# facebookresearch/videoseal

Hardware: AMD Instinct MI355X
Metric: frames/sec embed+extract 256-bit @768x768 (higher is better)
Workload: dtype f32 (2 x f16 operand split, 3 products on v_mfma_f32_32x32x16_f16, fp32 accumulate); 1 GPU; videoseal_1.0 256-bit, 32 frames 768x768 per GPU, image mode (embedder on every frame, full-res JND), embed + detect; card=videoseal_1.0, weights=random-init (seeded), no checkpoint offline, batch_per_gpu=32, mode=image

## Files before the change

### videoseal_amd/csrc/conv3x3_pl.hip

```cpp
#include <type_traits>

#include "conv_common.h"
#include "lds_dma.h"

int vs_splitk_epilogue(const vs_conv_desc_t& d, int M, hipStream_t st);

namespace {

using namespace vsconv;

constexpr int PT = 16, PPW = PT + 2, PPIX = PPW * PPW;
constexpr int PL_UNITS = PPIX * 2;
constexpr int P_DMAS = (2 * PL_UNITS + 63) / 64;
constexpr int P_BYTES = P_DMAS * 1024;
constexpr int Q_BYTES = 256 * 2 * 2 * 16;
constexpr int QX_OFF = 2 * P_BYTES;
constexpr int RING_OFF = QX_OFF + 2 * Q_BYTES;
constexpr int NRING = 6;

__device__ __forceinline__ void dma16(const char* gp, unsigned char* lds_base) { vs_lds_dma16(gp, lds_base); }
template <int N>
__device__ __forceinline__ void wait_vm() { asm volatile("s_waitcnt vmcnt(%0)" ::"n"(N) : "memory"); }

template <int TN>
__global__ __launch_bounds__(512, 2) void conv3x3_pl_kernel(const vs_conv_desc_t d, const int tiles_x, const int tiles_y, const int mtiles,
                                                            const int ntiles, const int cps) {
  using AR = Arith<2>;
  constexpr int TM = 2;
  constexpr int BN = 2 * TN * 32;
  constexpr int NG = BN / 32;
  constexpr int WBLK = 2048;
  constexpr int B_STAGE = NG * WBLK;
  __shared__ __attribute__((aligned(16))) unsigned char smem[RING_OFF + NRING * B_STAGE];
  unsigned char* const Bring = smem + RING_OFF;

  const int tid = threadIdx.x;
  const int lane = tid & 63;
  const int wave = __builtin_amdgcn_readfirstlane(tid >> 6);
  const int r = lane & 31, g = lane >> 5;

  const int bm = blockIdx.x % mtiles;
  const int bn = (blockIdx.x / mtiles) % ntiles;
  const int ks = blockIdx.x / (mtiles * ntiles);
  const int n0 = bn * BN;
  const int tx = bm % tiles_x;
  const int ty = (bm / tiles_x) % tiles_y;
  const int fb = bm / (tiles_x * tiles_y);
  const int y0 = ty * PT, x0 = tx * PT;

  const int spt_all = d.CinP / BK;
  const int sk = d.split_k > 1 ? d.split_k : 1;
  const bool p2_slice = sk > 1 && ks == sk;
  const int c_off = (sk > 1 && !p2_slice) ? ks * cps : 0;
  const int spt = p2_slice ? 0 : (sk > 1 ? min(cps, spt_all - c_off) : spt_all);
  const int n1 = 9 * spt;
  const int n2 = (d.in2_pl && (sk == 1 || p2_slice)) ? d.Cin2P / BK : 0;
  const int64_t Mpix = (int64_t)d.B * d.H * d.W;
  const int abl = VS_KERNEL_ABL(d);

  const int64_t cstride = Mpix * 32;
  const int pw = wave & 3;
  const int g0 = n0 / 32;
  const int ngroups = (d.N + 31) / 32;
  unsigned doff[6];
  unsigned pvalid = 0;
  int wdst[TN];
#pragma unroll
  for (int jj = 0; jj < TN; ++jj) {
    const int idx = pw * TN + jj;
    const int p = idx / NG, gi = idx - p * NG;
    wdst[jj] = __builtin_amdgcn_readfirstlane(p * (BN * 32) + gi * 1024);
  }
  auto weight_off = [&](const int nst) __attribute__((always_inline)) {
#pragma unroll
    for (int jj = 0; jj < TN; ++jj) {
      const int idx = pw * TN + jj;
      const int p = idx / NG, gi = idx - p * NG;
      const int gs = (g0 + gi) < ngroups ? g0 + gi : ngroups - 1;
      doff[jj] = (unsigned)(gs * nst) * WBLK + p * 1024 + lane * 16;
    }
  };
  const char* wbase = reinterpret_cast<const char*>(d.wt_blk) + (int64_t)c_off * 9 * WBLK;
  if (wave < 4) {
    weight_off(9 * spt_all);
  } else {
    const unsigned pstride = (unsigned)(spt_all * cstride);
#pragma unroll
    for (int j = 0; j < 6; ++j) {
      const int U = (pw + 4 * j) * 64 + lane;
      const int plane = U >= PL_UNITS ? 1 : 0;
      const int u = U - plane * PL_UNITS;
      const int q = u >> 1;
      const int py = q / PPW, px = q - py * PPW;
      const int hs = (u & 1) ^ (py & 1);
      const int iy = y0 - 1 + py, ix = x0 - 1 + px;
      const bool ok = U < 2 * PL_UNITS && iy >= 0 && iy < d.H && ix >= 0 && ix < d.W;
      doff[j] = ok ? plane * pstride + (unsigned)(((fb * d.H + iy) * d.W + ix) * 32 + hs * 16) : 0u;
      pvalid |= ok ? 1u << j : 0u;
      if (!ok && pw + 4 * j < P_DMAS) {
        *reinterpret_cast<u32x4*>(smem + (pw + 4 * j) * 1024 + lane * 16) = u32x4{0u, 0u, 0u, 0u};
        *reinterpret_cast<u32x4*>(smem + P_BYTES + (pw + 4 * j) * 1024 + lane * 16) = u32x4{0u, 0u, 0u, 0u};
      }
    }
  }
  int wstage = 0;
  auto dma_w2 = [&]() __attribute__((always_inline)) {
    unsigned char* st = Bring + wstage * B_STAGE;
#pragma unroll
    for (int jj = 0; jj < TN; ++jj) dma16(wbase + doff[jj], st + wdst[jj]);
    wbase += WBLK;
    wstage = wstage + 1 == NRING ? 0 : wstage + 1;
  };
  auto dma_w = [&](auto stagec) __attribute__((always_inline)) {
    unsigned char* st = Bring + decltype(stagec)::value * B_STAGE;
#pragma unroll
    for (int jj = 0; jj < TN; ++jj) dma16(wbase + doff[jj], st + wdst[jj]);
    wbase += WBLK;
  };
  const char* const inpl = reinterpret_cast<const char*>(d.in_pl);
  auto dma_patch2 = [&](const int cc, const int j0) __attribute__((always_inline)) {
    unsigned char* pb = smem + (cc & 1) * P_BYTES + pw * 1024;
    const char* cbase = inpl + (c_off + cc) * cstride;
#pragma unroll
    for (int jj = 0; jj < 2; ++jj) {
      const int j = j0 + jj;
      if (pw + 4 * j < P_DMAS) {
        if ((pvalid >> j) & 1) dma16(cbase + doff[j], pb + j * 4096);
      }
    }
  };
  auto qbuf = [&](const int c2) __attribute__((always_inline)) -> unsigned char* {
    const int b = c2 & 3;
    return smem + (b < 2 ? QX_OFF + b * Q_BYTES : (b - 2) * Q_BYTES);
  };
  const char* qbase = reinterpret_cast<const char*>(d.in2_pl);
  auto q_off = [&]() __attribute__((always_inline)) {
    const unsigned pstride2 = (unsigned)((d.Cin2P / BK) * cstride);
#pragma unroll
    for (int j = 0; j < 4; ++j) {
      const int U = (pw + 4 * j) * 64 + lane;
      const int plane = U >> 9;
      const int u = U & 511;
      const int p = u >> 1;
      const int hs = (u & 1) ^ ((p >> 3) & 1);
      const int iy = y0 + (p >> 4), ix = x0 + (p & 15);
      doff[j] = plane * pstride2 + (unsigned)(((fb * d.H + iy) * d.W + ix) * 32 + hs * 16);
    }
  };
  auto dma_q = [&](const int c2) __attribute__((always_inline)) {
    unsigned char* qb = qbuf(c2) + pw * 1024;
#pragma unroll
    for (int j = 0; j < 4; ++j) dma16(qbase + doff[j], qb + j * 4096);
    qbase += cstride;
  };

  const int wm = wave >> 1, wn = wave & 1;
  f32x16 acc[TM][TN];
#pragma unroll
  for (int i = 0; i < TM; ++i)
#pragma unroll
    for (int j = 0; j < TN; ++j)
#pragma unroll
      for (int e = 0; e < 16; ++e) acc[i][j][e] = 0.f;
  int q0[TM], p0[TM], prow[TM];
#pragma unroll
  for (int i = 0; i < TM; ++i) {
    p0[i] = (wm * TM + i) * 32 + r;
    q0[i] = (p0[i] >> 4) * PPW + (p0[i] & 15);
    prow[i] = (p0[i] >> 4) & 1;
  }
  const int b_frag = (wn * TN) * 1024 + (2 * r + (g ^ ((r >> 3) & 1))) * 16;

  struct Hi { bf16x8 a[TM]; bf16x8 b[TN]; };
  Hi H0, H1;
  bf16x8 lo_a[TM], lo_b[TN];
  auto b_ptr = [&](const int s) __attribute__((always_inline)) -> const unsigned char* { return Bring + (s % NRING) * B_STAGE + b_frag; };
  auto load_all2 = [&](Hi& H, const int c2) __attribute__((always_inline)) {
    const unsigned char* Bb = b_ptr(c2);
#pragma unroll
    for (int j = 0; j < TN; ++j) {
      H.b[j] = *reinterpret_cast<const bf16x8*>(Bb + j * 1024);
      lo_b[j] = *reinterpret_cast<const bf16x8*>(Bb + BN * 32 + j * 1024);
    }
    const unsigned char* Qs = qbuf(c2);
#pragma unroll
    for (int i = 0; i < TM; ++i) {
      const int ao = (2 * p0[i] + (g ^ ((p0[i] >> 3) & 1))) * 16;
      H.a[i] = *reinterpret_cast<const bf16x8*>(Qs + ao);
      lo_a[i] = *reinterpret_cast<const bf16x8*>(Qs + 512 * 16 + ao);
    }
  };
  auto mfma_q0 = [&](const Hi& H) __attribute__((always_inline)) {
#pragma unroll
    for (int i = 0; i < TM; ++i)
#pragma unroll
      for (int j = 0; j < TN; ++j) acc[i][j] = AR::mfma(H.b[j], lo_a[i], acc[i][j]);
  };
  auto mfma_q1 = [&](const Hi& H) __attribute__((always_inline)) {
#pragma unroll
    for (int i = 0; i < TM; ++i)
#pragma unroll
      for (int j = 0; j < TN; ++j) acc[i][j] = AR::mfma(lo_b[j], H.a[i], acc[i][j]);
  };
  auto mfma_q2 = [&](const Hi& H) __attribute__((always_inline)) {
#pragma unroll
    for (int i = 0; i < TM; ++i)
#pragma unroll
      for (int j = 0; j < TN; ++j) acc[i][j] = AR::mfma(H.b[j], H.a[i], acc[i][j]);
  };
  int ab[TM];
#pragma unroll
  for (int i = 0; i < TM; ++i) ab[i] = (2 * q0[i] + (g ^ prow[i])) * 16;
  auto ld_hi = [&](Hi& H, auto parc, auto tapc) __attribute__((always_inline)) {
    constexpr int PAR = decltype(parc)::value, TAP = decltype(tapc)::value;
    constexpr int ky = TAP / 3, kx = TAP % 3, STAGE = (PAR * 3 + TAP) % NRING;
    const unsigned char* Bb = Bring + STAGE * B_STAGE + b_frag;
#pragma unroll
    for (int j = 0; j < TN; ++j) H.b[j] = *reinterpret_cast<const bf16x8*>(Bb + j * 1024);
    const unsigned char* Ps = smem + PAR * P_BYTES + (ky * PPW + kx) * 32;
#pragma unroll
    for (int i = 0; i < TM; ++i) H.a[i] = *reinterpret_cast<const bf16x8*>(Ps + ((ky & 1) ? (ab[i] ^ 16) : ab[i]));
  };
  auto ld_alo = [&](auto parc, auto tapc) __attribute__((always_inline)) {
    constexpr int PAR = decltype(parc)::value, TAP = decltype(tapc)::value;
    constexpr int ky = TAP / 3, kx = TAP % 3;
    const unsigned char* Ps = smem + PAR * P_BYTES + PL_UNITS * 16 + (ky * PPW + kx) * 32;
#pragma unroll
    for (int i = 0; i < TM; ++i) lo_a[i] = *reinterpret_cast<const bf16x8*>(Ps + ((ky & 1) ? (ab[i] ^ 16) : ab[i]));
  };
  auto ld_blo = [&](auto parc, auto tapc) __attribute__((always_inline)) {
    constexpr int PAR = decltype(parc)::value, TAP = decltype(tapc)::value;
    constexpr int STAGE = (PAR * 3 + TAP) % NRING;
    const unsigned char* Bb = Bring + STAGE * B_STAGE + BN * 32 + b_frag;
#pragma unroll
    for (int j = 0; j < TN; ++j) lo_b[j] = *reinterpret_cast<const bf16x8*>(Bb + j * 1024);
  };
  using P0 = std::integral_constant<int, 0>;
  using P1 = std::integral_constant<int, 1>;
  auto tapstep = [&](auto parc, auto tapc, const int cc, const bool last) __attribute__((always_inline)) {
    constexpr int PAR = decltype(parc)::value, TAP = decltype(tapc)::value;
    constexpr bool ODD = ((PAR + TAP) & 1) != 0;
    const Hi& Hc = ODD ? H1 : H0;
    Hi& Hn = ODD ? H0 : H1;
    const int s = cc * 9 + TAP;
    mfma_q0(Hc);
    __builtin_amdgcn_sched_barrier(0);
    if (wave < 4) {
      if (s + NRING - 1 < n1) dma_w(std::integral_constant<int, (PAR * 3 + TAP + NRING - 1) % NRING>{});
    } else if constexpr (TAP < 3) {
      if (!last) dma_patch2(cc + 1, 2 * TAP);
    }
    if constexpr (TAP < 8) {
      ld_hi(Hn, parc, std::integral_constant<int, TAP + 1>{});
      ld_alo(parc, std::integral_constant<int, TAP + 1>{});
    } else if (!last) {
      ld_hi(Hn, std::integral_constant<int, 1 - PAR>{}, P0{});
      ld_alo(std::integral_constant<int, 1 - PAR>{}, P0{});
    }
    mfma_q1(Hc);
    __builtin_amdgcn_sched_barrier(0);
    if constexpr (TAP < 8) ld_blo(parc, std::integral_constant<int, TAP + 1>{});
    else if (!last) ld_blo(std::integral_constant<int, 1 - PAR>{}, P0{});
    mfma_q2(Hc);
    if (wave < 4) {
      if (s + NRING - 1 < n1) wait_vm<(NRING - 3) * TN>();
      else wait_vm<0>();
    } else if constexpr (TAP == 7) {
      if (!last) wait_vm<0>();
    }
    __builtin_amdgcn_s_waitcnt(0xC07F);
    __builtin_amdgcn_s_barrier();
  };
  auto chunk = [&](auto parc, const int cc) __attribute__((always_inline)) {
    const bool last = cc + 1 >= spt;
    tapstep(parc, std::integral_constant<int, 0>{}, cc, last);
    tapstep(parc, std::integral_constant<int, 1>{}, cc, last);
    tapstep(parc, std::integral_constant<int, 2>{}, cc, last);
    tapstep(parc, std::integral_constant<int, 3>{}, cc, last);
    tapstep(parc, std::integral_constant<int, 4>{}, cc, last);
    tapstep(parc, std::integral_constant<int, 5>{}, cc, last);
    tapstep(parc, std::integral_constant<int, 6>{}, cc, last);
    tapstep(parc, std::integral_constant<int, 7>{}, cc, last);
    tapstep(parc, std::integral_constant<int, 8>{}, cc, last);
  };

  if (spt > 0) {
  if (wave < 4) {
    dma_w(std::integral_constant<int, 0>{});
    dma_w(std::integral_constant<int, 1>{});
    dma_w(std::integral_constant<int, 2>{});
    dma_w(std::integral_constant<int, 3>{});
    dma_w(std::integral_constant<int, 4>{});
  } else {
    dma_patch2(0, 0);
    dma_patch2(0, 2);
    dma_patch2(0, 4);
  }
  wait_vm<0>();
  __builtin_amdgcn_s_barrier();

  ld_hi(H0, P0{}, P0{});
  ld_alo(P0{}, P0{});
  ld_blo(P0{}, P0{});
  __builtin_amdgcn_s_waitcnt(0xC07F);
  for (int cc = 0; cc < spt; cc += 2) {
    chunk(P0{}, cc);
    if (cc + 1 < spt) chunk(P1{}, cc + 1);
  }
  }
  int lane_e = lane;
  asm volatile("" : "+v"(lane_e));
  const int r_e = lane_e & 31, g_e = lane_e >> 5;
  int cbase[TN];
#pragma unroll
  for (int j = 0; j < TN; ++j) cbase[j] = n0 + (wn * TN + j) * 32 + 4 * g_e;
  auto ld4 = [](const float* p, int n, int N) __attribute__((always_inline)) -> f32x4 {
    f32x4 v = {0.f, 0.f, 0.f, 0.f};
    if (p) {
      if (n + 4 <= N) v = *reinterpret_cast<const f32x4*>(p + n);
      else
#pragma unroll
        for (int e = 0; e < 4; ++e)
          if (n + e < N) v[e] = p[n + e];
    }
    return v;
  };
  auto grp = [&](int i, int j, int q) __attribute__((always_inline)) -> f32x4 {
    return f32x4{acc[i][j][4 * q], acc[i][j][4 * q + 1], acc[i][j][4 * q + 2], acc[i][j][4 * q + 3]};
  };
  auto put = [&](int i, int j, int q, const f32x4& v) __attribute__((always_inline)) {
    acc[i][j][4 * q] = v[0]; acc[i][j][4 * q + 1] = v[1]; acc[i][j][4 * q + 2] = v[2]; acc[i][j][4 * q + 3] = v[3];
  };
  int64_t mrow[TM];
  int pcls[TM];
#pragma unroll
  for (int i = 0; i < TM; ++i) {
    const int pe = (wm * TM + i) * 32 + r_e;
    const int y = y0 + (pe >> 4), x = x0 + (pe & 15);
    mrow[i] = ((int64_t)fb * d.H + y) * d.W + x;
    pcls[i] = (y == 0 ? 0 : (y >= d.H - 1 ? 2 : 1)) * 3 + (x == 0 ? 0 : (x >= d.W - 1 ? 2 : 1));
  }
  scale_all<TM, TN>(acc, d.acc_mul);
  const bool full = n0 + BN <= d.N;
  if (sk == 1) {
    const float* tb = (d.tile_hint & VS_CONV_PRE) ? d.a_scale + (int64_t)fb * d.a_scale_ld : nullptr;
    const int64_t b2off = (int64_t)fb * d.bias2_fs;
    if (full && d.bias && (n2 == 0 || d.bias2)) {
#pragma unroll
      for (int j = 0; j < TN; ++j) {
        f32x4 b1[4], tv[TM][4];
#pragma unroll
        for (int q = 0; q < 4; ++q) b1[q] = *reinterpret_cast<const f32x4*>(d.bias + cbase[j] + 8 * q);
        if (tb) {
#pragma unroll
          for (int i = 0; i < TM; ++i)
#pragma unroll
            for (int q = 0; q < 4; ++q) tv[i][q] = *reinterpret_cast<const f32x4*>(tb + pcls[i] * d.N + cbase[j] + 8 * q);
        }
#pragma unroll
        for (int q = 0; q < 4; ++q)
#pragma unroll
          for (int i = 0; i < TM; ++i) {
            f32x4 v = grp(i, j, q) + b1[q];
            if (tb) v += tv[i][q];
            put(i, j, q, v);
          }
        __builtin_amdgcn_sched_barrier(0);
      }
      auto act_tile = [&](auto actc) __attribute__((always_inline)) {
        constexpr int ACT = decltype(actc)::value;
#pragma unroll
        for (int i = 0; i < TM; ++i)
#pragma unroll
          for (int j = 0; j < TN; ++j)
#pragma unroll
            for (int e = 0; e < 16; ++e) acc[i][j][e] = vs_apply_act(acc[i][j][e], ACT < 0 ? d.act : ACT);
      };
      if (d.act == VS_ACT_RELU) act_tile(std::integral_constant<int, VS_ACT_RELU>{});
      else if (d.act != VS_ACT_NONE) act_tile(std::integral_constant<int, -1>{});
#pragma unroll
      for (int j = 0; j < TN; ++j) {
        f32x4 b2[4];
#pragma unroll
        for (int q = 0; q < 4; ++q) b2[q] = n2 > 0 ? *reinterpret_cast<const f32x4*>(d.bias2 + b2off + cbase[j] + 8 * q) : f32x4{0.f, 0.f, 0.f, 0.f};
#pragma unroll
        for (int q = 0; q < 4; ++q)
#pragma unroll
          for (int i = 0; i < TM; ++i) put(i, j, q, grp(i, j, q) + b2[q]);
      }
    } else {
#pragma unroll
    for (int j = 0; j < TN; ++j)
#pragma unroll
      for (int q = 0; q < 4; ++q) {
        const int n = cbase[j] + 8 * q;
        const f32x4 b1 = ld4(d.bias, n, d.N);
        const f32x4 b2 = n2 > 0 ? ld4(d.bias2 ? d.bias2 + b2off : nullptr, n, d.N) : f32x4{0.f, 0.f, 0.f, 0.f};
#pragma unroll
        for (int i = 0; i < TM; ++i) {
          f32x4 v = grp(i, j, q) + b1;
          if (tb) v += ld4(tb + pcls[i] * d.N, n, d.N);
#pragma unroll
          for (int e = 0; e < 4; ++e) v[e] = vs_apply_act(v[e], d.act);
          put(i, j, q, v + b2);
        }
      }
    }
  }
  if (n2 > 0) {
    scale_all<TM, TN>(acc, 1.f / d.acc_mul2);
    wstage = 0;
    wbase = reinterpret_cast<const char*>(d.wt2_blk);
    if (wave < 4) {
      weight_off(n2);
      for (int t = 0; t < NRING - 1 && t < n2; ++t) dma_w2();
    } else {
      q_off();
      for (int c = 0; c < 3 && c < n2; ++c) dma_q(c);
    }
    wait_vm<0>();
    __builtin_amdgcn_s_barrier();
    for (int c2 = 0; c2 < n2; ++c2) {
      if (wave < 4) {
        if (c2 + NRING - 1 < n2) dma_w2();
      } else if (c2 + 3 < n2) {
        dma_q(c2 + 3);
      }
      load_all2(H0, c2);
      mfma_q0(H0);
      mfma_q1(H0);
      mfma_q2(H0);
      if (wave < 4) {
        if (c2 + NRING - 1 < n2) wait_vm<(NRING - 3) * TN>();
        else wait_vm<0>();
      } else {
        const int allow = min(n2 - 1, c2 + 3) - (c2 + 1);
        if (allow >= 2) wait_vm<8>();
        else if (allow == 1) wait_vm<4>();
        else wait_vm<0>();
      }
      __builtin_amdgcn_s_waitcnt(0xC07F);
      __builtin_amdgcn_s_barrier();
    }
    scale_all<TM, TN>(acc, d.acc_mul2);
  }
  if (abl & 32) return;
  if (sk > 1) {
    float* ws = d.splitk_ws + (int64_t)ks * Mpix * d.splitk_ld;
#pragma unroll
    for (int i = 0; i < TM; ++i)
#pragma unroll
      for (int j = 0; j < TN; ++j)
#pragma unroll
        for (int q = 0; q < 4; ++q) {
          const int n = cbase[j] + 8 * q;
          if (n < d.N) *reinterpret_cast<f32x4*>(ws + mrow[i] * d.splitk_ld + n) = grp(i, j, q);
        }
    return;
  }
  auto store_all = [&](auto fullc) __attribute__((always_inline)) {
    constexpr bool FULL = decltype(fullc)::value;
#pragma unroll
    for (int i = 0; i < TM; ++i) {
      float* orow = d.out ? d.out + mrow[i] * d.out_ld + d.out_coff : nullptr;
      const float* rrow = d.res ? d.res + mrow[i] * d.res_ld : nullptr;
      f32x4 rv[TN][4];
      if constexpr (FULL) {
        if (rrow) {
#pragma unroll
          for (int j = 0; j < TN; ++j)
#pragma unroll
            for (int q = 0; q < 4; ++q) rv[j][q] = *reinterpret_cast<const f32x4*>(rrow + cbase[j] + 8 * q);
        }
      }
      char* prow = d.out_pl ? reinterpret_cast<char*>(d.out_pl) + mrow[i] * 32 : nullptr;
      const int64_t opstride = (int64_t)(d.N / BK) * cstride;
#pragma unroll
      for (int j = 0; j < TN; ++j)
#pragma unroll
        for (int q2 = 0; q2 < 2; ++q2) {
          f32x4 v[2];
#pragma unroll
          for (int h = 0; h < 2; ++h) {
            const int n = cbase[j] + 8 * (2 * q2 + h);
            if constexpr (FULL) {
              v[h] = grp(i, j, 2 * q2 + h);
              if (rrow) v[h] += rv[j][2 * q2 + h];
            } else {
              v[h] = f32x4{0.f, 0.f, 0.f, 0.f};
              if (n >= d.n_store) continue;
              if (n < d.N) {
                v[h] = grp(i, j, 2 * q2 + h);
                if (rrow) v[h] += *reinterpret_cast<const f32x4*>(rrow + n);
                if (n + 4 > d.N)
#pragma unroll
                  for (int e = 0; e < 4; ++e)
                    if (n + e >= d.N) v[h][e] = 0.f;
              }
            }
            if (orow) *reinterpret_cast<f32x4*>(orow + n) = v[h];
          }
          const int n16 = n0 + (wn * TN + j) * 32 + 16 * q2;
          if (prow && (FULL || n16 < d.N)) {
            u32x2 h0, l0, h1, l1;
            split4h(v[0], d.a_mul, h0, l0);
            split4h(v[1], d.a_mul, h1, l1);
            const auto sh0 = __builtin_amdgcn_permlane32_swap(h0[0], h1[0], false, false);
            const auto sh1 = __builtin_amdgcn_permlane32_swap(h0[1], h1[1], false, false);
            const auto sl0 = __builtin_amdgcn_permlane32_swap(l0[0], l1[0], false, false);
            const auto sl1 = __builtin_amdgcn_permlane32_swap(l0[1], l1[1], false, false);
            char* dst = prow + (int64_t)(n16 >> 4) * cstride + g_e * 16;
            *reinterpret_cast<u32x4*>(dst) = u32x4{sh0[0], sh1[0], sh0[1], sh1[1]};
            *reinterpret_cast<u32x4*>(dst + opstride) = u32x4{sl0[0], sl1[0], sl0[1], sl1[1]};
          }
        }
    }
  };
  if (full) store_all(std::true_type{});
  else store_all(std::false_type{});
}

__global__ __launch_bounds__(256) void to_planes_kernel(const float* __restrict__ x, const int64_t rows, const int C, const int64_t ld,
                                                        const float a_mul, char* __restrict__ pl) {
  const int64_t idx = (int64_t)blockIdx.x * 256 + threadIdx.x;
  const int64_t per_chunk = rows * 2;
  const int chunks = C / 16;
  if (idx >= per_chunk * chunks) return;
  const int c = (int)(idx / per_chunk);
  const int64_t rem = idx - (int64_t)c * per_chunk;
  const int64_t row = rem >> 1;
  const int h = (int)(rem & 1);
  const float* src = x + row * ld + c * 16 + h * 8;
  const f32x4 a = *reinterpret_cast<const f32x4*>(src), b = *reinterpret_cast<const f32x4*>(src + 4);
  u32x2 ah, al, bh, bl;
  split4h(a, a_mul, ah, al);
  split4h(b, a_mul, bh, bl);
  char* dst = pl + ((int64_t)c * rows + row) * 32 + h * 16;
  *reinterpret_cast<u32x4*>(dst) = u32x4{ah[0], ah[1], bh[0], bh[1]};
  *reinterpret_cast<u32x4*>(dst + (int64_t)chunks * rows * 32) = u32x4{al[0], al[1], bl[0], bl[1]};
}

template <int TN>
int launch_pl(const vs_conv_desc_t& d, hipStream_t st) {
  constexpr int BN = 2 * TN * 32;
  const int tiles_x = d.W / PT, tiles_y = d.H / PT;
  const int sk = d.split_k > 1 ? d.split_k : 1;
  const int64_t mt = (int64_t)d.B * tiles_x * tiles_y, nt = cdiv64(sk > 1 ? d.N : d.n_store, BN);
  const int spt = d.CinP / BK;
  const int cps = (spt + sk - 1) / sk;
  if (sk > 1 && (int64_t)(sk - 1) * cps >= spt) return VS_ERR_BAD_ARG;
  const int slices = sk > 1 ? sk + (d.in2_pl ? 1 : 0) : 1;
  if (mt * nt * slices > 0x7fffffffLL) return VS_ERR_UNSUPPORTED;
  hipLaunchKernelGGL((conv3x3_pl_kernel<TN>), dim3((unsigned)(mt * nt * slices)), dim3(512), 0, st, d, tiles_x, tiles_y, (int)mt, (int)nt, cps);
  int rc = vs_launch_status();
  if (rc != VS_OK || sk == 1) return rc;
  return vs_splitk_epilogue(d, (int)((int64_t)d.B * d.H * d.W), st);
}

}

int vs_conv3x3_pl_dispatch(const vs_conv_desc_t& d, int tile, hipStream_t st) {
  switch (tile) {
    case 22: return launch_pl<3>(d, st);
    case 23: return launch_pl<2>(d, st);
    default: return VS_ERR_UNSUPPORTED;
  }
}

extern "C" int vs_to_planes(const float* x, int64_t rows, int C, int64_t ld, float a_mul, void* planes, void* stream) {
  VS_REQUIRE(x && planes && rows > 0 && C > 0 && C % 16 == 0 && ld >= C && ld % 4 == 0 && a_mul > 0.f);
  VS_REQUIRE(((uintptr_t)x & 15) == 0 && ((uintptr_t)planes & 15) == 0);
  const int64_t items = rows * 2 * (C / 16);
  hipLaunchKernelGGL(to_planes_kernel, dim3((unsigned)cdiv64(items, 256)), dim3(256), 0, (hipStream_t)stream, x, rows, C, ld, a_mul,
                     static_cast<char*>(planes));
  return vs_launch_status();
}
```

Measured before the change: 4271 frames/s.

## Add specialized epilogue forms for common conv3x3 planes configurations

Adds compile-time specialized kernel instances (planes out, planes out with second-input pass, f32 out with second-input pass) chosen on the host when the conv has bias, ReLU, no split-K, no residual and full N tiles. The specialized epilogue preloads bias vectors, fuses scale, bias, ReLU, bias2 and the inverse second scale into one pass, and issues the pass-2 DMA prefetch before that arithmetic so the loads overlap it. The aim is to cut runtime branching and register pressure in the epilogue and to hide pass-2 load latency, at the cost of more kernel instances and a launch-count atomic counter.

After: 4291 frames/s, median of 6. About the same (+0.5%).

```diff
diff --git a/videoseal_amd/csrc/conv3x3_pl.hip b/videoseal_amd/csrc/conv3x3_pl.hip
--- a/videoseal_amd/csrc/conv3x3_pl.hip
+++ b/videoseal_amd/csrc/conv3x3_pl.hip
@@ -1,3 +1,4 @@
+#include <atomic>
 #include <type_traits>
 
 #include "conv_common.h"
@@ -17,15 +18,17 @@
 constexpr int QX_OFF = 2 * P_BYTES;
 constexpr int RING_OFF = QX_OFF + 2 * Q_BYTES;
 constexpr int NRING = 6;
+enum { PL_GENERAL = 0, PL_PLANES = 1, PL_PLANES_P2 = 2, PL_F32_P2 = 3, PL_FORMS = 4 };
 
 __device__ __forceinline__ void dma16(const char* gp, unsigned char* lds_base) { vs_lds_dma16(gp, lds_base); }
 template <int N>
 __device__ __forceinline__ void wait_vm() { asm volatile("s_waitcnt vmcnt(%0)" ::"n"(N) : "memory"); }
 
-template <int TN>
-__global__ __launch_bounds__(512, 2) void conv3x3_pl_kernel(const vs_conv_desc_t d, const int tiles_x, const int tiles_y, const int mtiles,
-                                                            const int ntiles, const int cps) {
+template <int TN, int FORM>
+__device__ __forceinline__ void pl_body(const vs_conv_desc_t d, const int tiles_x, const int tiles_y, const int mtiles, const int ntiles, const int cps,
+                                        const float inv_mul2) {
   using AR = Arith<2>;
+  constexpr bool SPEC = FORM != PL_GENERAL;
   constexpr int TM = 2;
   constexpr int BN = 2 * TN * 32;
   constexpr int NG = BN / 32;
@@ -49,14 +52,14 @@
   const int y0 = ty * PT, x0 = tx * PT;
 
   const int spt_all = d.CinP / BK;
-  const int sk = d.split_k > 1 ? d.split_k : 1;
+  const int sk = (!SPEC && d.split_k > 1) ? d.split_k : 1;
   const bool p2_slice = sk > 1 && ks == sk;
   const int c_off = (sk > 1 && !p2_slice) ? ks * cps : 0;
   const int spt = p2_slice ? 0 : (sk > 1 ? min(cps, spt_all - c_off) : spt_all);
   const int n1 = 9 * spt;
-  const int n2 = (d.in2_pl && (sk == 1 || p2_slice)) ? d.Cin2P / BK : 0;
+  const int n2 = SPEC ? (FORM == PL_PLANES ? 0 : d.Cin2P / BK) : (d.in2_pl && (sk == 1 || p2_slice)) ? d.Cin2P / BK : 0;
   const int64_t Mpix = (int64_t)d.B * d.H * d.W;
-  const int abl = VS_KERNEL_ABL(d);
+  const int abl = SPEC ? 0 : VS_KERNEL_ABL(d);
 
   const int64_t cstride = Mpix * 32;
   const int pw = wave & 3;
@@ -308,107 +311,7 @@
     if (cc + 1 < spt) chunk(P1{}, cc + 1);
   }
   }
-  int lane_e = lane;
-  asm volatile("" : "+v"(lane_e));
-  const int r_e = lane_e & 31, g_e = lane_e >> 5;
-  int cbase[TN];
-#pragma unroll
-  for (int j = 0; j < TN; ++j) cbase[j] = n0 + (wn * TN + j) * 32 + 4 * g_e;
-  auto ld4 = [](const float* p, int n, int N) __attribute__((always_inline)) -> f32x4 {
-    f32x4 v = {0.f, 0.f, 0.f, 0.f};
-    if (p) {
-      if (n + 4 <= N) v = *reinterpret_cast<const f32x4*>(p + n);
-      else
-#pragma unroll
-        for (int e = 0; e < 4; ++e)
-          if (n + e < N) v[e] = p[n + e];
-    }
-    return v;
-  };
-  auto grp = [&](int i, int j, int q) __attribute__((always_inline)) -> f32x4 {
-    return f32x4{acc[i][j][4 * q], acc[i][j][4 * q + 1], acc[i][j][4 * q + 2], acc[i][j][4 * q + 3]};
-  };
-  auto put = [&](int i, int j, int q, const f32x4& v) __attribute__((always_inline)) {
-    acc[i][j][4 * q] = v[0]; acc[i][j][4 * q + 1] = v[1]; acc[i][j][4 * q + 2] = v[2]; acc[i][j][4 * q + 3] = v[3];
-  };
-  int64_t mrow[TM];
-  int pcls[TM];
-#pragma unroll
-  for (int i = 0; i < TM; ++i) {
-    const int pe = (wm * TM + i) * 32 + r_e;
-    const int y = y0 + (pe >> 4), x = x0 + (pe & 15);
-    mrow[i] = ((int64_t)fb * d.H + y) * d.W + x;
-    pcls[i] = (y == 0 ? 0 : (y >= d.H - 1 ? 2 : 1)) * 3 + (x == 0 ? 0 : (x >= d.W - 1 ? 2 : 1));
-  }
-  scale_all<TM, TN>(acc, d.acc_mul);
-  const bool full = n0 + BN <= d.N;
-  if (sk == 1) {
-    const float* tb = (d.tile_hint & VS_CONV_PRE) ? d.a_scale + (int64_t)fb * d.a_scale_ld : nullptr;
-    const int64_t b2off = (int64_t)fb * d.bias2_fs;
-    if (full && d.bias && (n2 == 0 || d.bias2)) {
-#pragma unroll
-      for (int j = 0; j < TN; ++j) {
-        f32x4 b1[4], tv[TM][4];
-#pragma unroll
-        for (int q = 0; q < 4; ++q) b1[q] = *reinterpret_cast<const f32x4*>(d.bias + cbase[j] + 8 * q);
-        if (tb) {
-#pragma unroll
-          for (int i = 0; i < TM; ++i)
-#pragma unroll
-            for (int q = 0; q < 4; ++q) tv[i][q] = *reinterpret_cast<const f32x4*>(tb + pcls[i] * d.N + cbase[j] + 8 * q);
-        }
-#pragma unroll
-        for (int q = 0; q < 4; ++q)
-#pragma unroll
-          for (int i = 0; i < TM; ++i) {
-            f32x4 v = grp(i, j, q) + b1[q];
-            if (tb) v += tv[i][q];
-            put(i, j, q, v);
-          }
-        __builtin_amdgcn_sched_barrier(0);
-      }
-      auto act_tile = [&](auto actc) __attribute__((always_inline)) {
-        constexpr int ACT = decltype(actc)::value;
-#pragma unroll
-        for (int i = 0; i < TM; ++i)
-#pragma unroll
-          for (int j = 0; j < TN; ++j)
-#pragma unroll
-            for (int e = 0; e < 16; ++e) acc[i][j][e] = vs_apply_act(acc[i][j][e], ACT < 0 ? d.act : ACT);
-      };
-      if (d.act == VS_ACT_RELU) act_tile(std::integral_constant<int, VS_ACT_RELU>{});
-      else if (d.act != VS_ACT_NONE) act_tile(std::integral_constant<int, -1>{});
-#pragma unroll
-      for (int j = 0; j < TN; ++j) {
-        f32x4 b2[4];
-#pragma unroll
-        for (int q = 0; q < 4; ++q) b2[q] = n2 > 0 ? *reinterpret_cast<const f32x4*>(d.bias2 + b2off + cbase[j] + 8 * q) : f32x4{0.f, 0.f, 0.f, 0.f};
-#pragma unroll
-        for (int q = 0; q < 4; ++q)
-#pragma unroll
-          for (int i = 0; i < TM; ++i) put(i, j, q, grp(i, j, q) + b2[q]);
-      }
-    } else {
-#pragma unroll
-    for (int j = 0; j < TN; ++j)
-#pragma unroll
-      for (int q = 0; q < 4; ++q) {
-        const int n = cbase[j] + 8 * q;
-        const f32x4 b1 = ld4(d.bias, n, d.N);
-        const f32x4 b2 = n2 > 0 ? ld4(d.bias2 ? d.bias2 + b2off : nullptr, n, d.N) : f32x4{0.f, 0.f, 0.f, 0.f};
-#pragma unroll
-        for (int i = 0; i < TM; ++i) {
-          f32x4 v = grp(i, j, q) + b1;
-          if (tb) v += ld4(tb + pcls[i] * d.N, n, d.N);
-#pragma unroll
-          for (int e = 0; e < 4; ++e) v[e] = vs_apply_act(v[e], d.act);
-          put(i, j, q, v + b2);
-        }
-      }
-    }
-  }
-  if (n2 > 0) {
-    scale_all<TM, TN>(acc, 1.f / d.acc_mul2);
+  auto p2_fill = [&]() __attribute__((always_inline)) {
     wstage = 0;
     wbase = reinterpret_cast<const char*>(d.wt2_blk);
     if (wave < 4) {
@@ -418,8 +321,8 @@
       q_off();
       for (int c = 0; c < 3 && c < n2; ++c) dma_q(c);
     }
-    wait_vm<0>();
-    __builtin_amdgcn_s_barrier();
+  };
+  auto p2_loop = [&]() __attribute__((always_inline)) {
     for (int c2 = 0; c2 < n2; ++c2) {
       if (wave < 4) {
         if (c2 + NRING - 1 < n2) dma_w2();
@@ -442,6 +345,189 @@
       __builtin_amdgcn_s_waitcnt(0xC07F);
       __builtin_amdgcn_s_barrier();
     }
+  };
+  if constexpr (SPEC) {
+    constexpr bool P2 = FORM != PL_PLANES, F32 = FORM == PL_F32_P2;
+    int lane_s = lane;
+    asm volatile("" : "+v"(lane_s));
+    const int r_s = lane_s & 31, g_s = lane_s >> 5;
+    const int cb0 = n0 + wn * TN * 32 + 4 * g_s;
+    f32x4 bv[TN][4];
+#pragma unroll
+    for (int j = 0; j < TN; ++j)
+#pragma unroll
+      for (int q = 0; q < 4; ++q) bv[j][q] = *reinterpret_cast<const f32x4*>(d.bias + cb0 + 32 * j + 8 * q);
+    const float m1 = d.acc_mul;
+    if constexpr (P2) {
+      const float* b2p = d.bias2 + (int64_t)fb * d.bias2_fs + cb0;
+      f32x4 b2v[TN][4];
+#pragma unroll
+      for (int j = 0; j < TN; ++j)
+#pragma unroll
+        for (int q = 0; q < 4; ++q) b2v[j][q] = *reinterpret_cast<const f32x4*>(b2p + 32 * j + 8 * q);
+      p2_fill();
+#pragma unroll
+      for (int j = 0; j < TN; ++j) {
+#pragma unroll
+        for (int i = 0; i < TM; ++i)
+#pragma unroll
+          for (int e = 0; e < 16; ++e)
+            acc[i][j][e] = (vs_apply_act(acc[i][j][e] * m1 + bv[j][e >> 2][e & 3], VS_ACT_RELU) + b2v[j][e >> 2][e & 3]) * inv_mul2;
+        __builtin_amdgcn_sched_barrier(0);
+      }
+      wait_vm<0>();
+      __builtin_amdgcn_s_barrier();
+      p2_loop();
+    }
+    const float m2 = d.acc_mul2, a_mul = d.a_mul;
+    const int64_t opstride = (int64_t)(d.N / BK) * cstride;
+    char* rowp[TM];
+#pragma unroll
+    for (int i = 0; i < TM; ++i) {
+      const int pe = (wm * TM + i) * 32 + r_s;
+      const int64_t m = ((int64_t)fb * d.H + y0 + (pe >> 4)) * d.W + x0 + (pe & 15);
+      if constexpr (F32) rowp[i] = reinterpret_cast<char*>(d.out + m * d.out_ld + d.out_coff + cb0);
+      else rowp[i] = reinterpret_cast<char*>(d.out_pl) + m * 32 + g_s * 16 + (int64_t)(n0 / 16 + wn * TN * 2) * cstride;
+    }
+#pragma unroll
+    for (int i = 0; i < TM; ++i)
+#pragma unroll
+      for (int j = 0; j < TN; ++j) {
+#pragma unroll
+        for (int q2 = 0; q2 < 2; ++q2) {
+          f32x4 v[2];
+#pragma unroll
+          for (int h = 0; h < 2; ++h)
+#pragma unroll
+            for (int e = 0; e < 4; ++e) {
+              const float a = acc[i][j][8 * q2 + 4 * h + e];
+              v[h][e] = P2 ? a * m2 : vs_apply_act(a * m1 + bv[j][2 * q2 + h][e], VS_ACT_RELU);
+            }
+          if constexpr (F32) {
+            *reinterpret_cast<f32x4*>(rowp[i] + (32 * j + 16 * q2) * 4) = v[0];
+            *reinterpret_cast<f32x4*>(rowp[i] + (32 * j + 16 * q2 + 8) * 4) = v[1];
+          } else {
+            u32x2 h0, l0, h1, l1;
+            split4h(v[0], a_mul, h0, l0);
+            split4h(v[1], a_mul, h1, l1);
+            const auto sh0 = __builtin_amdgcn_permlane32_swap(h0[0], h1[0], false, false);
+            const auto sh1 = __builtin_amdgcn_permlane32_swap(h0[1], h1[1], false, false);
+            const auto sl0 = __builtin_amdgcn_permlane32_swap(l0[0], l1[0], false, false);
+            const auto sl1 = __builtin_amdgcn_permlane32_swap(l0[1], l1[1], false, false);
+            char* dst = rowp[i] + (2 * j + q2) * cstride;
+            *reinterpret_cast<u32x4*>(dst) = u32x4{sh0[0], sh1[0], sh0[1], sh1[1]};
+            *reinterpret_cast<u32x4*>(dst + opstride) = u32x4{sl0[0], sl1[0], sl0[1], sl1[1]};
+          }
+        }
+        __builtin_amdgcn_sched_barrier(0);
+      }
+    return;
+  }
+  int lane_e = lane;
+  asm volatile("" : "+v"(lane_e));
+  const int r_e = lane_e & 31, g_e = lane_e >> 5;
+  int cbase[TN];
+#pragma unroll
+  for (int j = 0; j < TN; ++j) cbase[j] = n0 + (wn * TN + j) * 32 + 4 * g_e;
+  auto ld4 = [](const float* p, int n, int N) __attribute__((always_inline)) -> f32x4 {
+    f32x4 v = {0.f, 0.f, 0.f, 0.f};
+    if (p) {
+      if (n + 4 <= N) v = *reinterpret_cast<const f32x4*>(p + n);
+      else
+#pragma unroll
+        for (int e = 0; e < 4; ++e)
+          if (n + e < N) v[e] = p[n + e];
+    }
+    return v;
+  };
+  auto grp = [&](int i, int j, int q) __attribute__((always_inline)) -> f32x4 {
+    return f32x4{acc[i][j][4 * q], acc[i][j][4 * q + 1], acc[i][j][4 * q + 2], acc[i][j][4 * q + 3]};
+  };
+  auto put = [&](int i, int j, int q, const f32x4& v) __attribute__((always_inline)) {
+    acc[i][j][4 * q] = v[0]; acc[i][j][4 * q + 1] = v[1]; acc[i][j][4 * q + 2] = v[2]; acc[i][j][4 * q + 3] = v[3];
+  };
+  int64_t mrow[TM];
+  int pcls[TM];
+#pragma unroll
+  for (int i = 0; i < TM; ++i) {
+    const int pe = (wm * TM + i) * 32 + r_e;
+    const int y = y0 + (pe >> 4), x = x0 + (pe & 15);
+    mrow[i] = ((int64_t)fb * d.H + y) * d.W + x;
+    pcls[i] = (y == 0 ? 0 : (y >= d.H - 1 ? 2 : 1)) * 3 + (x == 0 ? 0 : (x >= d.W - 1 ? 2 : 1));
+  }
+  scale_all<TM, TN>(acc, d.acc_mul);
+  const bool full = n0 + BN <= d.N;
+  if (sk == 1) {
+    const float* tb = (d.tile_hint & VS_CONV_PRE) ? d.a_scale + (int64_t)fb * d.a_scale_ld : nullptr;
+    const int64_t b2off = (int64_t)fb * d.bias2_fs;
+    if (full && d.bias && (n2 == 0 || d.bias2)) {
+#pragma unroll
+      for (int j = 0; j < TN; ++j) {
+        f32x4 b1[4], tv[TM][4];
+#pragma unroll
+        for (int q = 0; q < 4; ++q) b1[q] = *reinterpret_cast<const f32x4*>(d.bias + cbase[j] + 8 * q);
+        if (tb) {
+#pragma unroll
+          for (int i = 0; i < TM; ++i)
+#pragma unroll
+            for (int q = 0; q < 4; ++q) tv[i][q] = *reinterpret_cast<const f32x4*>(tb + pcls[i] * d.N + cbase[j] + 8 * q);
+        }
+#pragma unroll
+        for (int q = 0; q < 4; ++q)
+#pragma unroll
+          for (int i = 0; i < TM; ++i) {
+            f32x4 v = grp(i, j, q) + b1[q];
+            if (tb) v += tv[i][q];
+            put(i, j, q, v);
+          }
+        __builtin_amdgcn_sched_barrier(0);
+      }
+      auto act_tile = [&](auto actc) __attribute__((always_inline)) {
+        constexpr int ACT = decltype(actc)::value;
+#pragma unroll
+        for (int i = 0; i < TM; ++i)
+#pragma unroll
+          for (int j = 0; j < TN; ++j)
+#pragma unroll
+            for (int e = 0; e < 16; ++e) acc[i][j][e] = vs_apply_act(acc[i][j][e], ACT < 0 ? d.act : ACT);
+      };
+      if (d.act == VS_ACT_RELU) act_tile(std::integral_constant<int, VS_ACT_RELU>{});
+      else if (d.act != VS_ACT_NONE) act_tile(std::integral_constant<int, -1>{});
+#pragma unroll
+      for (int j = 0; j < TN; ++j) {
+        f32x4 b2[4];
+#pragma unroll
+        for (int q = 0; q < 4; ++q) b2[q] = n2 > 0 ? *reinterpret_cast<const f32x4*>(d.bias2 + b2off + cbase[j] + 8 * q) : f32x4{0.f, 0.f, 0.f, 0.f};
+#pragma unroll
+        for (int q = 0; q < 4; ++q)
+#pragma unroll
+          for (int i = 0; i < TM; ++i) put(i, j, q, grp(i, j, q) + b2[q]);
+      }
+    } else {
+#pragma unroll
+    for (int j = 0; j < TN; ++j)
+#pragma unroll
+      for (int q = 0; q < 4; ++q) {
+        const int n = cbase[j] + 8 * q;
+        const f32x4 b1 = ld4(d.bias, n, d.N);
+        const f32x4 b2 = n2 > 0 ? ld4(d.bias2 ? d.bias2 + b2off : nullptr, n, d.N) : f32x4{0.f, 0.f, 0.f, 0.f};
+#pragma unroll
+        for (int i = 0; i < TM; ++i) {
+          f32x4 v = grp(i, j, q) + b1;
+          if (tb) v += ld4(tb + pcls[i] * d.N, n, d.N);
+#pragma unroll
+          for (int e = 0; e < 4; ++e) v[e] = vs_apply_act(v[e], d.act);
+          put(i, j, q, v + b2);
+        }
+      }
+    }
+  }
+  if (n2 > 0) {
+    scale_all<TM, TN>(acc, 1.f / d.acc_mul2);
+    p2_fill();
+    wait_vm<0>();
+    __builtin_amdgcn_s_barrier();
+    p2_loop();
     scale_all<TM, TN>(acc, d.acc_mul2);
   }
   if (abl & 32) return;
@@ -520,6 +606,18 @@
   else store_all(std::false_type{});
 }
 
+template <int TN>
+__global__ __launch_bounds__(512, 2) void conv3x3_pl_kernel(const vs_conv_desc_t d, const int tiles_x, const int tiles_y, const int mtiles,
+                                                            const int ntiles, const int cps) {
+  pl_body<TN, PL_GENERAL>(d, tiles_x, tiles_y, mtiles, ntiles, cps, 0.f);
+}
+template <int TN, int FORM>
+__global__ __launch_bounds__(512, 2) void conv3x3_pl_kernel_form(const vs_conv_desc_t d, const int tiles_x, const int tiles_y, const int mtiles,
+                                                                 const int ntiles, const float inv_mul2) {
+  static_assert(FORM != PL_GENERAL, "the general instance is conv3x3_pl_kernel");
+  pl_body<TN, FORM>(d, tiles_x, tiles_y, mtiles, ntiles, 0, inv_mul2);
+}
+
 __global__ __launch_bounds__(256) void to_planes_kernel(const float* __restrict__ x, const int64_t rows, const int C, const int64_t ld,
                                                         const float a_mul, char* __restrict__ pl) {
   const int64_t idx = (int64_t)blockIdx.x * 256 + threadIdx.x;
@@ -541,6 +639,18 @@
 }
 
 template <int TN>
+int pl_form(const vs_conv_desc_t& d) {
+  constexpr int BN = 2 * TN * 32;
+  if (TN != 3) return PL_GENERAL;
+  if (d.split_k > 1 || VS_KERNEL_ABL(d) != 0 || !d.bias || d.bias_fs != 0 || d.act != VS_ACT_RELU || d.res || (d.tile_hint & VS_CONV_PRE)) return PL_GENERAL;
+  if (d.N % BN != 0 || d.n_store != d.N || (d.out != nullptr) == (d.out_pl != nullptr)) return PL_GENERAL;
+  if (!d.in2_pl) return d.out_pl ? PL_PLANES : PL_GENERAL;
+  if (!d.bias2) return PL_GENERAL;
+  return d.out_pl ? PL_PLANES_P2 : PL_F32_P2;
+}
+std::atomic<long long> g_form_launches[PL_FORMS];
+
+template <int TN>
 int launch_pl(const vs_conv_desc_t& d, hipStream_t st) {
   constexpr int BN = 2 * TN * 32;
   const int tiles_x = d.W / PT, tiles_y = d.H / PT;
@@ -551,7 +661,19 @@
   if (sk > 1 && (int64_t)(sk - 1) * cps >= spt) return VS_ERR_BAD_ARG;
   const int slices = sk > 1 ? sk + (d.in2_pl ? 1 : 0) : 1;
   if (mt * nt * slices > 0x7fffffffLL) return VS_ERR_UNSUPPORTED;
-  hipLaunchKernelGGL((conv3x3_pl_kernel<TN>), dim3((unsigned)(mt * nt * slices)), dim3(512), 0, st, d, tiles_x, tiles_y, (int)mt, (int)nt, cps);
+  const int form = pl_form<TN>(d);
+  const float inv_mul2 = form >= PL_PLANES_P2 ? 1.f / d.acc_mul2 : 0.f;
+  const dim3 grid((unsigned)(mt * nt * slices));
+  if constexpr (TN == 3) {
+    auto go = [&](auto formc) {
+      hipLaunchKernelGGL((conv3x3_pl_kernel_form<TN, decltype(formc)::value>), grid, dim3(512), 0, st, d, tiles_x, tiles_y, (int)mt, (int)nt, inv_mul2);
+    };
+    if (form == PL_PLANES) go(std::integral_constant<int, PL_PLANES>{});
+    else if (form == PL_PLANES_P2) go(std::integral_constant<int, PL_PLANES_P2>{});
+    else if (form == PL_F32_P2) go(std::integral_constant<int, PL_F32_P2>{});
+  }
+  if (form == PL_GENERAL) hipLaunchKernelGGL((conv3x3_pl_kernel<TN>), grid, dim3(512), 0, st, d, tiles_x, tiles_y, (int)mt, (int)nt, cps);
+  g_form_launches[form].fetch_add(1, std::memory_order_relaxed);
   int rc = vs_launch_status();
   if (rc != VS_OK || sk == 1) return rc;
   return vs_splitk_epilogue(d, (int)((int64_t)d.B * d.H * d.W), st);
@@ -565,6 +687,10 @@
     case 23: return launch_pl<2>(d, st);
     default: return VS_ERR_UNSUPPORTED;
   }
+}
+
+extern "C" long long vs_conv3x3_pl_form_launches(int form) {
+  return form >= 0 && form < PL_FORMS ? g_form_launches[form].load(std::memory_order_relaxed) : -1;
 }
 
 extern "C" int vs_to_planes(const float* x, int64_t rows, int C, int64_t ld, float a_mul, void* planes, void* stream) {
```
